# JialeTao/MRFA

Hardware: AMD Instinct MI355X
Metric: frames/sec (256x256 source+driving pair) fwd+bwd (higher is better)
Workload: dtype f32; 1 GPU; vox1.yaml MTIA (TokenPose_B) prior + DenseMotion + RaftFlow refinement, 256x256, bs=8/GPU, fwd+bwd+clip+Adam, train-mode BN, surrogate L1 loss; global_batch=8, parallelism=dp1, prior=mtia, background_predictor=False, sync_bn=False, launch=hipGraph, optimizer=FlatAdam (K20), mfma=bf16x6

## Files before the change

### mrfa_amd/build.py

```python
import glob
import os
import subprocess
import sys

HERE = os.path.dirname(os.path.abspath(__file__))
ROOT = os.path.dirname(HERE)
CSRC = os.path.join(HERE, "csrc")
LIBDIR = os.path.join(HERE, "_lib")
LIB = os.path.join(LIBDIR, "libmrfa_hip.so")
SOURCES = ["error.cpp", "conv_plan.hip", "conv_mfma.hip", "conv_split.hip", "conv_halo.hip", "conv_small.hip", "conv_lean.hip", "wgrad_mfma.hip", "wgrad_split.hip", "wgrad_halo.hip", "wgrad_small.hip", "wgrad_lean.hip", "conv_fewout.hip", "conv_fewout3.hip", "layout.hip", "pack_multi.hip", "norm.hip", "sample.hip", "elementwise.hip", "optim.hip", "tokenpose.hip", "attention_mfma.hip", "losses.hip", "prior.hip", "pose.hip"]
FLAGS = ["--offload-arch=gfx950", "-O3", "-std=c++17", "-fPIC", "-I" + os.path.join(ROOT, "include"), "-I" + CSRC,
         "-Wno-unused-result"]


def _stale(out, deps):
    if not os.path.exists(out):
        return True
    t = os.path.getmtime(out)
    return any(os.path.getmtime(d) > t for d in deps)


def build(force: bool = False, verbose: bool = True) -> str:
    os.makedirs(LIBDIR, exist_ok=True)
    hipcc = os.environ.get("HIPCC", "/opt/rocm/bin/hipcc")
    headers = [os.path.join(ROOT, "include", h) for h in ("mrfa_hip.h", "mrfa_hip_ext.h")] + sorted(glob.glob(os.path.join(CSRC, "*.h")))
    objs = []
    procs = []
    for src in SOURCES:
        sp = os.path.join(CSRC, src)
        if not os.path.exists(sp):
            raise FileNotFoundError(sp)
        obj = os.path.join(LIBDIR, os.path.splitext(src)[0] + ".o")
        objs.append(obj)
        if force or _stale(obj, [sp] + headers):
            cmd = [hipcc] + FLAGS + (["-x", "hip"] if src.endswith(".cpp") else []) + ["-c", sp, "-o", obj]
            if verbose:
                print("[mrfa_amd.build]", " ".join(cmd), flush=True)
            procs.append((src, subprocess.Popen(cmd)))
    for src, pr in procs:
        if pr.wait() != 0:
            raise RuntimeError(f"hipcc failed on {src}")
    if force or _stale(LIB, objs):
        cmd = [hipcc, "--offload-arch=gfx950", "-shared", "-fPIC", "-o", LIB] + objs
        if verbose:
            print("[mrfa_amd.build]", " ".join(cmd), flush=True)
        subprocess.check_call(cmd)
    return LIB


if __name__ == "__main__":
    build(force="--force" in sys.argv)
    print(LIB)
```

### mrfa_amd/csrc/common.h

```cpp
#pragma once
#include <hip/hip_runtime.h>
#include <stdio.h>
#include <string.h>
#include "mrfa_hip.h"

typedef float f32x16 __attribute__((ext_vector_type(16)));
typedef float f32x4 __attribute__((ext_vector_type(4)));

void mrfa_set_error(const char* fmt, ...);

struct MrfaTuning {
    int conv_small_env;
    int conv_small;
    int conv_halo, conv_halo_min_tiles, conv_halo_pr, conv_halo_phase, conv_halo_bn256, conv_halo_bn192, conv_halo_bn64_fill;
    int conv_lean, conv_lean_min_wgs, conv_lean_geo, gemm_lean;
    int wgrad_halo, wgrad_halo_min_wgs, wgrad_halo_target_wgs, wgrad_halo_phase, wgrad_lean;
    int conv_fewout3, attention_mfma, split_target_256;
};
extern MrfaTuning g_tune;

struct HaloGeo { int PR, BN; bool phase; };

enum class ConvFamily { lean, gemm_lean, small, halo, halo_dgrad, rows_split, rows_f32, refused };
struct ConvPlan {
    ConvFamily family;
    char error[256];
    long long M;
    int KT;
    int lean_geo, gemm_cfg, small_tm, small_tn;
    HaloGeo halo;
    int BM, BN, splitk;
    bool w8;
    bool fused;
    bool fin_in_launch;
    bool reads_w;
    int last_config;
    bool groups_ok, bst_ok, stride2_ok, mask_ok, phase_dgrad_ok;
};
ConvPlan plan_conv(const mrfa_conv_params& p);

enum class WgradFamily { lean, small, halo, tiled, refused };
struct WgradPlan {
    WgradFamily family;
    char error[192];
    long long M;
    bool lean, small;
    bool groups_ok, stride2_ok;
};
WgradPlan plan_wgrad(const mrfa_wgrad_params& p);

int mrfa_conv_split_launch(hipStream_t st, const mrfa_conv_params& p, int KT, long long M, int splitk, int BN);
bool mrfa_conv_halo_eligible(const mrfa_conv_params& p, HaloGeo* geo);
int mrfa_conv_halo_launch(hipStream_t st, const mrfa_conv_params& p, const HaloGeo& geo);
int mrfa_wgrad_split_launch(hipStream_t st, const mrfa_wgrad_params& p, dim3 grid, long long M, long long kps, int tiles_n, int nsplit, int inner,
                            int total_splits, int taps, long long partial_stride, int BM, int BN);

bool mrfa_wgrad_halo_eligible(const mrfa_wgrad_params& p);
int mrfa_wgrad_halo_launch(hipStream_t st, const mrfa_wgrad_params& p);

bool mrfa_fewout3_wgrad(hipStream_t st, const float* x, int ldx, int N, int H, int W, int Cin, const float* dy, int lddy, int Cout, int R, int pad,
                        float* dw, float* dbias, int* rc);

int mrfa_conv_lean_pick(const mrfa_conv_params& p);
int mrfa_conv_lean_launch(hipStream_t st, const mrfa_conv_params& p, int geo);
int mrfa_gemm_lean_pick(const mrfa_conv_params& p, long long M);
int mrfa_gemm_lean_launch(hipStream_t st, const mrfa_conv_params& p, long long M, int cfg);

bool mrfa_conv_small_eligible(const mrfa_conv_params& p, long long M);
int mrfa_conv_small_launch(hipStream_t st, const mrfa_conv_params& p, long long M, int tm, int tn);

bool mrfa_attention_mfma_ok(int d, int n, const void* qkv, int ld, const void* out, int ldo, const void* dout, int lddo, const void* dqkv, int lddq);
int mrfa_attention_fwd_mfma(hipStream_t st, const float* qkv, int ld, int B, int n, int heads, int d, float scale, float* out, int ldo, float* lse);
int mrfa_attention_bwd_mfma(hipStream_t st, const float* qkv, int ld, const float* out, int ldo, const float* dout, int lddo, const float* lse,
                            float* delta, int B, int n, int heads, int d, float scale, float* dqkv, int lddq);

bool mrfa_wgrad_lean_eligible(const mrfa_wgrad_params& p);
int mrfa_wgrad_lean_multi(hipStream_t st, const mrfa_wgrad_params* ps, int n, unsigned char* taken);

bool mrfa_wgrad_small_eligible(const mrfa_wgrad_params& p, long long M);
int mrfa_wgrad_small_launch(hipStream_t st, const mrfa_wgrad_params& p, long long M);

#define MRFA_CHECK_ARG(cond, ...)                      \
    do {                                               \
        if (!(cond)) {                                 \
            mrfa_set_error(__VA_ARGS__);               \
            return 1;                                  \
        }                                              \
    } while (0)

#define MRFA_CHECK_LAUNCH(name)                                                   \
    do {                                                                          \
        hipError_t e_ = hipGetLastError();                                        \
        if (e_ != hipSuccess) {                                                   \
            mrfa_set_error("%s: launch failed: %s", name, hipGetErrorString(e_)); \
            return 2;                                                             \
        }                                                                         \
    } while (0)

static inline bool aligned16(const void* p) { return (reinterpret_cast<uintptr_t>(p) & 15u) == 0; }
static inline int cdiv(long long a, long long b) { return (int)((a + b - 1) / b); }

static inline int stream_grid(long long work_items, int block) {
    long long g = (work_items + block - 1) / block;
    if (g < 1) g = 1;
    if (g > 256 * 16) g = 256 * 16;
    return (int)g;
}

__device__ __forceinline__ int xcd_tile_index() {
    const int per_xcd = (int)gridDim.x >> 3;
    return (int)(blockIdx.x & 7) * per_xcd + (int)(blockIdx.x >> 3);
}

__device__ __forceinline__ void chain_prio() {
    __builtin_amdgcn_s_setprio(3);
}

__device__ __forceinline__ int stat_group(const mrfa_conv_params& p, long long row, long long M) {
    return p.groups > 1 ? (int)(row / (M / p.groups)) : 0;
}
__device__ __forceinline__ double* stat_slot(const mrfa_conv_params& p, int group, unsigned slot) {
    return p.stats + ((size_t)group * MRFA_STATS_SLOTS + slot % MRFA_STATS_SLOTS) * 2 * p.Cout;
}
static inline long long group_rows(const mrfa_conv_params& p, long long M) {
    if (p.groups <= 1) return M;
    return (p.N % p.groups) == 0 ? M / p.groups : 0;
}

__device__ __forceinline__ bool splitk_last_arriver(unsigned* ticket, unsigned nsplit) {
    __shared__ unsigned s_sk_ticket;
    asm volatile("s_waitcnt vmcnt(0)" ::: "memory");
    __syncthreads();
    if (threadIdx.x == 0) s_sk_ticket = __hip_atomic_fetch_add(ticket, 1u, __ATOMIC_RELAXED, __HIP_MEMORY_SCOPE_AGENT);
    __syncthreads();
    return s_sk_ticket == nsplit - 1;
}

__device__ __forceinline__ bool fin_last_arriver(unsigned* counter, unsigned participants, int idx) {
    __shared__ unsigned s_fin_ticket;
    asm volatile("s_waitcnt vmcnt(0)" ::: "memory");
    __syncthreads();
    if (threadIdx.x == 0) {
        if (idx < 0) {
            s_fin_ticket = __hip_atomic_fetch_add(counter, 1u, __ATOMIC_RELAXED, __HIP_MEMORY_SCOPE_AGENT) == participants - 1;
        } else {
            const unsigned nsh = participants < 8u ? participants : 8u, sh = (unsigned)idx % nsh;
            const unsigned mine = participants / nsh + (sh < participants % nsh ? 1u : 0u);
            unsigned last = 0;
            if (__hip_atomic_fetch_add(counter + 1 + sh, 1u, __ATOMIC_RELAXED, __HIP_MEMORY_SCOPE_AGENT) == mine - 1)
                last = __hip_atomic_fetch_add(counter, 1u, __ATOMIC_RELAXED, __HIP_MEMORY_SCOPE_AGENT) == nsh - 1;
            s_fin_ticket = last;
        }
    }
    __syncthreads();
    return s_fin_ticket != 0;
}

__device__ __forceinline__ double fin_slot_sum(const double* first, size_t stride) {
    double v[MRFA_STATS_SLOTS];
#pragma unroll
    for (int s = 0; s < MRFA_STATS_SLOTS; ++s) v[s] = __hip_atomic_load(first + (size_t)s * stride, __ATOMIC_RELAXED, __HIP_MEMORY_SCOPE_AGENT);
    double t = 0.0;
#pragma unroll
    for (int s = 0; s < MRFA_STATS_SLOTS; ++s) t += v[s];
    return t;
}

__device__ __forceinline__ void fused_bn_finalize(const mrfa_conv_params& p, unsigned participants, int idx = -1, double* scratch = nullptr, int scratch_n = 0) {
    if (!fin_last_arriver(p.fin_counter, participants, idx)) return;
    const double cnt = (double)p.fin_count;
    const int G = p.groups > 1 ? p.groups : 1;
    const int C2 = 2 * p.Cout;
    const bool par = scratch != nullptr && scratch_n >= G * C2;
    if (par) {
        for (int o = threadIdx.x; o < G * C2; o += blockDim.x) scratch[o] = fin_slot_sum(p.stats + (size_t)(o / C2) * MRFA_STATS_SLOTS * C2 + o % C2, (size_t)C2);
        __syncthreads();
    }
    for (int c = threadIdx.x; c < p.Cout; c += blockDim.x) {
        float rm = p.fin_rmean ? p.fin_rmean[c] : 0.f, rv = p.fin_rmean ? p.fin_rvar[c] : 0.f;
        for (int g = 0; g < G; ++g) {
            const double* sg = p.stats + (size_t)g * MRFA_STATS_SLOTS * C2;
            const double t1 = par ? scratch[g * C2 + c] : fin_slot_sum(sg + c, (size_t)C2);
            const double t2 = par ? scratch[g * C2 + p.Cout + c] : fin_slot_sum(sg + p.Cout + c, (size_t)C2);
            const double m = t1 / cnt;
            double var = t2 / cnt - m * m;
            if (var < 0.0) var = 0.0;
            const float mean = (float)m, invstd = (float)(1.0 / sqrt(var + (double)p.fin_eps));
            const double unb = p.fin_count > 1 ? var * cnt / (cnt - 1.0) : var;
            rm = (1.f - p.fin_momentum) * rm + p.fin_momentum * mean;
            rv = (1.f - p.fin_momentum) * rv + p.fin_momentum * (float)unb;
            const float sc = p.fin_gamma[c] * invstd;
            const int gc = g * p.Cout + c;
            p.fin_scale[gc] = sc;
            p.fin_shift[gc] = p.fin_beta[c] - mean * sc;
            if (p.fin_mean) p.fin_mean[gc] = mean;
            if (p.fin_invstd) p.fin_invstd[gc] = invstd;
        }
        if (p.fin_rmean) { p.fin_rmean[c] = rm; p.fin_rvar[c] = rv; }
    }
}

__device__ __forceinline__ float wave_sum(float v) {
#pragma unroll
    for (int o = 32; o > 0; o >>= 1) v += __shfl_xor(v, o, 64);
    return v;
}
```

### mrfa_amd/csrc/conv_plan.hip

```cpp
#include "common.h"
#include <stdarg.h>
#include <stdlib.h>

namespace {
int env_int(const char* name, int dflt) { const char* e = getenv(name); return e ? atoi(e) : dflt; }
int env_on(const char* name) { const char* e = getenv(name); return !(e && e[0] == '0'); }
}

MrfaTuning g_tune = {
     env_on("MRFA_CONV_SMALL"),  1,
     env_on("MRFA_CONV_HALO"),  128,  0,  1,  1,
     1,  1,
     env_on("MRFA_CONV_LEAN"),  128,  -1,
     env_int("MRFA_GEMM_LEAN", 1),
     env_on("MRFA_WGRAD_HALO"),  192,  256,  1,
     env_on("MRFA_WGRAD_LEAN"),
     1,  env_on("MRFA_ATTENTION_MFMA"),  env_int("MRFA_SPLIT_TARGET_256", 1),
};

enum TuneKind { T_ON, T_INT, T_NONNEG, T_NONNEG_ON, T_LEVEL, T_POS };
static const struct { const char* key; int* field; TuneKind kind; } TUNING_KEYS[] = {
    {"conv_small", &g_tune.conv_small, T_ON},
    {"conv_halo", &g_tune.conv_halo, T_ON},
    {"conv_halo_min_tiles", &g_tune.conv_halo_min_tiles, T_INT},
    {"conv_halo_pr", &g_tune.conv_halo_pr, T_INT},
    {"conv_halo_phase", &g_tune.conv_halo_phase, T_ON},
    {"conv_halo_bn256", &g_tune.conv_halo_bn256, T_ON},
    {"conv_halo_bn192", &g_tune.conv_halo_bn192, T_ON},
    {"conv_halo_bn64_fill", &g_tune.conv_halo_bn64_fill, T_ON},
    {"conv_lean", &g_tune.conv_lean, T_ON},
    {"conv_lean_min_wgs", &g_tune.conv_lean_min_wgs, T_NONNEG},
    {"conv_lean_geo", &g_tune.conv_lean_geo, T_INT},
    {"gemm_lean", &g_tune.gemm_lean, T_LEVEL},
    {"wgrad_halo", &g_tune.wgrad_halo, T_ON},
    {"wgrad_halo_min_wgs", &g_tune.wgrad_halo_min_wgs, T_NONNEG},
    {"wgrad_halo_target_wgs", &g_tune.wgrad_halo_target_wgs, T_POS},
    {"wgrad_halo_phase", &g_tune.wgrad_halo_phase, T_NONNEG_ON},
    {"wgrad_lean", &g_tune.wgrad_lean, T_ON},
    {"conv_fewout3", &g_tune.conv_fewout3, T_ON},
    {"attention_mfma", &g_tune.attention_mfma, T_ON},
};

extern "C" int mrfa_set_tuning(const char* key, int value) {
    if (!key) return -1;
    for (const auto& k : TUNING_KEYS) {
        if (strcmp(key, k.key)) continue;
        const int prev = *k.field;
        switch (k.kind) {
            case T_ON: *k.field = value != 0; break;
            case T_INT: *k.field = value; break;
            case T_NONNEG: if (value >= 0) *k.field = value; break;
            case T_NONNEG_ON: if (value >= 0) *k.field = value != 0; break;
            case T_LEVEL: if (value >= 0) *k.field = value > 2 ? 2 : value; break;
            case T_POS: if (value > 0) *k.field = value; break;
        }
        return prev;
    }
    return -1;
}

namespace {
constexpr int BK = 32;

template <typename Plan>
Plan& refuse(Plan& c, const char* fmt, ...) {
    va_list ap;
    va_start(ap, fmt);
    vsnprintf(c.error, sizeof(c.error), fmt, ap);
    va_end(ap);
    c.family = decltype(c.family)::refused;
    return c;
}

void plan_rows(ConvPlan& c, const mrfa_conv_params& p, int mode) {
    const bool flat = p.kflat > 0;
    const long long M = c.M;
    const int KT = c.KT;
    const int nb = p.nbatch > 1 ? p.nbatch : 1;
    int BN = 128;
    {
        const int cands[4] = {128, 96, 64, 32};
        const double pen[4] = {1.0, 1.08, 1.16, 1.3};
        double best = 1e18;
        for (int i = 0; i < 4; ++i) {
            if (cands[i] == 96 && flat) continue;
            const double cost = (double)cdiv(p.Cout, cands[i]) * cands[i] * pen[i];
            if (cost < best) { best = cost; BN = cands[i]; }
        }
    }
    if (mode >= 1 && !flat && p.Cout >= 32) BN = p.Cout <= 64 ? 64 : 128;
    auto ntiles = [&](int bm, int bn) { return ((M + bm - 1) / bm) * cdiv(p.Cout, bn) * nb; };
    int BM = 128;
    if (BN == 96 && ntiles(128, 96) < 384) BN = 128;
    if (BN == 128) { if (M <= 32) BM = 32; else if (M <= 64) BM = 64; }
    else if (BN == 64 && M <= 64) BM = 64;
    int splitk = 1;
    const bool auto_split = (p.splitk == 0);
    if (p.splitk > 1) splitk = p.splitk;
    {
        const bool short_k_big_m = KT < 32 && M > 4096;
        const bool grouped_stats = p.groups > 1 && p.stats && !(p.sk_ticket && !p.accumulate);
        const int max_split = (auto_split && !short_k_big_m && !grouped_stats) ? (KT / 2 > 0 ? KT / 2 : 1) : 1;
        long long t = ntiles(BM, BN);
        if (t < 384 && !(short_k_big_m && t >= 128)) {
            const bool half_target = g_tune.split_target_256 && auto_split && p.sk_ticket && !p.accumulate && KT >= 72 && KT <= 320 && BM == 128 && t >= 8 && t <= 16;
            int want = (int)(((half_target ? 256 : 512) + t - 1) / t);
            if (auto_split) splitk = want <= max_split ? want : max_split;
            const int min_bm = (BN == 128) ? 32 : (BN == 64 ? 64 : 128);
            while (!half_target && ntiles(BM, BN) * splitk < 384 && BM > min_bm) {
                BM >>= 1;
                if (auto_split) {
                    t = ntiles(BM, BN);
                    want = (int)((512 + t - 1) / t);
                    splitk = want <= max_split ? want : max_split;
                }
            }
            if (splitk < 1) splitk = 1;
        }
    }
    bool w8 = false;
    if (p.tile) {
        BM = p.tile >> 16; BN = p.tile & 0x7fff; w8 = (p.tile & 0x8000) != 0;
        if (p.splitk >= 1) splitk = p.splitk;
    } else if (BM == 128 && BN == 128 && !flat) {
        w8 = true;
    }
    const bool split_operand = mode >= 1 && BM == 128 && (BN == 128 || BN == 64) && !flat;
    c.family = split_operand ? ConvFamily::rows_split : ConvFamily::rows_f32;
    c.BM = BM;
    c.BN = BN;
    c.w8 = w8;
    c.splitk = splitk;
    c.fused = splitk > 1 && p.sk_ticket && !p.accumulate;
    c.fin_in_launch = p.fin_scale && nb == 1 && (splitk == 1 || c.fused);
    c.reads_w = !(split_operand && mode != 3 && p.w_split);
    c.last_config = (BM << 16) | (BN << 4) | ((flat ? 1 : 0) << 1) | (splitk > 1 ? 1 : 0) | (split_operand ? 4 : 0);
}
}

ConvPlan plan_conv(const mrfa_conv_params& p) {
    ConvPlan c = {};
    const int mode = mrfa_get_mfma_mode();
    const bool flat = p.kflat > 0;
    c.M = (long long)p.N * p.Hout * p.Wout;
    c.KT = ((flat ? p.kflat : p.R * p.S * p.Cin) + BK - 1) / BK;
    c.splitk = 1;
    c.reads_w = true;
    c.fin_in_launch = p.fin_scale != nullptr;

    c.lean_geo = flat ? -1 : mrfa_conv_lean_pick(p);
    c.gemm_cfg = (flat || c.lean_geo >= 0) ? -1 : mrfa_gemm_lean_pick(p, c.M);
    const bool lean = c.lean_geo >= 0, gemm = c.gemm_cfg >= 0;
    const bool small = !lean && !gemm && g_tune.conv_small_env && g_tune.conv_small && mrfa_conv_small_eligible(p, c.M);
    const bool halo = !flat && mrfa_conv_halo_eligible(p, &c.halo);

    const long long rows = group_rows(p, c.M);
    c.groups_ok = p.groups <= 1 || !(p.stats || p.fin_scale || p.bst_x || p.in_scale) ||
                  (p.nbatch <= 1 && p.splitk <= 1 && rows > 0 &&
                   (lean || gemm || (!p.in_scale && ((rows % 128) == 0 || small || (p.stride <= 1 && halo)))));
    c.bst_ok = p.stats && !p.fin_scale && p.stride >= 0 && !flat && (lean || gemm || small);
    c.stride2_ok = p.stride == 2 && p.Hout == (p.Hin + 2 * p.pad - p.R) / 2 + 1 && p.Wout == (p.Win + 2 * p.pad - p.S) / 2 + 1 &&
                   (flat ? (!p.ups && p.nbatch <= 1 && p.splitk <= 1 && p.ktab) : small);
    c.mask_ok = halo;
    c.phase_dgrad_ok = p.ups == 2 && halo;

    if (!(p.x && p.w)) return refuse(c, "conv2d: null pointer");
    if (!(p.N > 0 && p.Cin > 0 && p.Cout > 0 && p.Hout > 0 && p.Wout > 0)) return refuse(c, "conv2d: bad sizes");
    if (!(p.R >= 1 && p.S >= 1 && p.R <= 15 && p.S <= 15)) return refuse(c, "conv2d: kernel size %dx%d unsupported", p.R, p.S);
    if (!((p.w_ld % 4) == 0 && aligned16(p.w))) return refuse(c, "conv2d: packed weight must be 16-B aligned, w_ld %% 4 == 0");
    if (!flat && (p.Cin % 32) != 0) return refuse(c, "conv2d: chunked mode needs Cin %% 32 == 0 (got %d); use flat mode", p.Cin);
    if (!flat && !((p.ldx % 4) == 0 && aligned16(p.x))) return refuse(c, "conv2d: chunked mode needs 16-B aligned x and ldx %% 4 == 0");
    if (!flat && p.in_scale && !(aligned16(p.in_scale) && aligned16(p.in_shift))) return refuse(c, "conv2d: in_scale/in_shift alignment");
    if (flat && !(p.ktab != nullptr && aligned16(p.ktab))) return refuse(c, "conv2d: flat mode needs a 16-B aligned ktab");
    if (lean) {
        c.family = ConvFamily::lean;
        c.reads_w = false;
        c.last_config = (32 << 16) | (32 << 4) | 4 | (1 << 27);
        return c;
    }
    if (gemm) {
        c.family = ConvFamily::gemm_lean;
        c.reads_w = false;
        c.last_config = (64 << 16) | (64 << 4) | 4 | (1 << 26);
        return c;
    }
    if (small) {
        c.family = ConvFamily::small;
        const int ncols = (p.Cout + 15) / 16 * 16;
        auto waves = [&](int wm, int wn) { return ((c.M + wm - 1) / wm) * ((ncols + wn - 1) / wn); };
        int tm = 2, tn = 2;
        if (waves(32, 32) < 2048) { tm = 1; tn = 2; }
        if (tm == 1 && waves(16, 32) < 2048) { tn = 1; }
        if (ncols % 32 != 0 && tn == 2 && ncols < 32) tn = 1;
        if (p.groups > 1 && tm == 2 && (rows % 128) != 0) tm = 1;
        c.small_tm = tm;
        c.small_tn = tn;
        c.last_config = (16 << 16) | (16 << 4) | 8;
        return c;
    }
    if (p.stride < 0 || p.stride > 2 || (p.stride == 2 && !(flat && !p.ups && p.nbatch <= 1)))
        return refuse(c, "conv2d: stride = %d is only implemented by the one-wave-per-tile kernel and by flat-K launches: ask mrfa_conv2d_stride_supported() first", p.stride);
    if (p.mask && !halo) return refuse(c, "conv2d: `mask` is only honoured by the patch-tiled kernel: ask mrfa_conv2d_mask_supported() first");
    if (p.ups == 2 && !halo)
        return refuse(c, "conv2d: ups = 2 (phase data gradient of a fused-upsample layer) is only implemented for the shapes mrfa_conv2d_phase_dgrad_supported() reports");
    if (halo) {
        c.family = p.ups == 2 ? ConvFamily::halo_dgrad : ConvFamily::halo;
        c.reads_w = false;
        c.last_config = (128 << 16) | ((p.Cout <= 64 ? 64 : 128) << 4) | 4 | (1 << 28);
        return c;
    }
    plan_rows(c, p, mode);
    return c;
}

WgradPlan plan_wgrad(const mrfa_wgrad_params& p) {
    WgradPlan c = {};
    const bool flat = p.kflat > 0;
    c.M = (long long)p.N * p.Hout * p.Wout;
    c.lean = mrfa_wgrad_lean_eligible(p);
    c.small = g_tune.conv_small_env && g_tune.conv_small && mrfa_wgrad_small_eligible(p, c.M);
    c.groups_ok = p.groups <= 1 || !p.in_scale || c.lean;
    c.stride2_ok = p.stride == 2 && p.Hout == (p.Hin + 2 * p.pad - p.R) / 2 + 1 && p.Wout == (p.Win + 2 * p.pad - p.S) / 2 + 1 && c.small;
    if (!(p.x && p.dy && p.dw)) return refuse(c, "wgrad: null pointer");
    if (!flat && !((p.ldx % 4) == 0 && aligned16(p.x))) return refuse(c, "wgrad: x must be a 16-B aligned view with ld %% 4 == 0");
    if (flat && !p.ktab) return refuse(c, "wgrad: flat mode needs ktab");
    if (!(c.M < (1ll << 31) - 64)) return refuse(c, "wgrad: too many pixels");
    if (p.in_scale && c.lean) { c.family = WgradFamily::lean; return c; }
    if (!c.groups_ok) return refuse(c, "wgrad: groups = %d with a prologue is only implemented where mrfa_conv2d_wgrad_groups_supported() says so", p.groups);
    if (c.small) { c.family = WgradFamily::small; return c; }
    if (p.stride > 1) return refuse(c, "wgrad: stride = %d is only implemented by the small-problem kernel: ask mrfa_conv2d_wgrad_stride_supported() first", p.stride);
    c.family = !flat && mrfa_wgrad_halo_eligible(p) ? WgradFamily::halo : WgradFamily::tiled;
    return c;
}

extern "C" int mrfa_conv2d_split_k(const mrfa_conv_params* p) {
    if (!p) return 1;
    if (p->splitk > 1) return p->splitk;
    const ConvPlan c = plan_conv(*p);
    return c.family == ConvFamily::refused ? 1 : c.splitk;
}

extern "C" int mrfa_conv2d_reads_fp32_weights(const mrfa_conv_params* p) {
    if (!p) return 1;
    const ConvPlan c = plan_conv(*p);
    return c.family == ConvFamily::refused || c.reads_w ? 1 : 0;
}

extern "C" int mrfa_conv2d_groups_supported(const mrfa_conv_params* p) { return p && plan_conv(*p).groups_ok ? 1 : 0; }
extern "C" int mrfa_conv2d_bwdstats_supported(const mrfa_conv_params* p) { return p && plan_conv(*p).bst_ok ? 1 : 0; }
extern "C" int mrfa_conv2d_stride_supported(const mrfa_conv_params* p) { return p && plan_conv(*p).stride2_ok ? 1 : 0; }
extern "C" int mrfa_conv2d_mask_supported(const mrfa_conv_params* p) { return p && plan_conv(*p).mask_ok ? 1 : 0; }
extern "C" int mrfa_conv2d_phase_dgrad_supported(const mrfa_conv_params* p) { return p && plan_conv(*p).phase_dgrad_ok ? 1 : 0; }

extern "C" int mrfa_conv2d_wgrad_stride_supported(const mrfa_wgrad_params* p) { return p && plan_wgrad(*p).stride2_ok ? 1 : 0; }
extern "C" int mrfa_conv2d_wgrad_groups_supported(const mrfa_wgrad_params* p) { return p && plan_wgrad(*p).groups_ok ? 1 : 0; }
extern "C" int mrfa_conv2d_wgrad_lean_supported(const mrfa_wgrad_params* p) { return p && plan_wgrad(*p).lean ? 1 : 0; }
```

### mrfa_amd/csrc/wgrad_small.hip

```cpp
#include <vector>
#include "common.h"

namespace {

typedef float f32x4v __attribute__((ext_vector_type(4)));
typedef float f32x2v __attribute__((ext_vector_type(2)));

struct SmallProblem {
    const float* x; const float* dy; float* dw; float* dbias;
    int ldx, ldy, Hin, Win, Hout, Wout, Cin, Cout, R, S, pad, stride;
    float alpha;
    int M, chunks_per_wave, nblk_ci, nblk, pow2_w , pow2_hw, workgroups, groups8 ;
};

template <bool SPATIAL, bool POW2, bool ROWS, int NT>
__device__ __forceinline__ void wgrad_small_body(const SmallProblem& p, const int g, const int tap, const int blk, float (*sacc)[16 * NT][16 * NT + 1], float* sbias) {
    typedef float VT __attribute__((ext_vector_type(NT)));
    constexpr int B = 16 * NT;
    const long long M = p.M;
    const int chunks_per_wave = p.chunks_per_wave, nblk_ci = p.nblk_ci, nblk = p.nblk, pow2_w = p.pow2_w, pow2_hw = p.pow2_hw;
    const int lane = threadIdx.x & 63, wave = threadIdx.x >> 6;
    const int li = lane & 15, kq = lane >> 4;
    const int co0 = (blk / nblk_ci) * B, ci0 = (blk % nblk_ci) * B;
    const int dr = tap / p.S - p.pad, ds = tap % p.S - p.pad;
    const int Mi = (int)M;
    const int range = (4 * g + wave) * chunks_per_wave * 16;
    const int HWo = p.Hout * p.Wout;
    const int wstride = p.stride > 1 ? p.stride : 1;

    if (threadIdx.x < B) sbias[threadIdx.x] = 0.f;
    __syncthreads();

    f32x4v acc[NT][NT];
#pragma unroll
    for (int t = 0; t < NT; ++t)
#pragma unroll
        for (int u = 0; u < NT; ++u) acc[t][u] = f32x4v{0.f, 0.f, 0.f, 0.f};
    float bsum[NT];
#pragma unroll
    for (int t = 0; t < NT; ++t) bsum[t] = 0.f;
    const VT vzero = {};
    const float* dyp = p.dy + co0 + NT * li;
    const float* xp = p.x + ci0 + NT * li;

    int dy_lane[4], x_lane[4];
#pragma unroll
    for (int j = 0; j < 4; ++j) {
        dy_lane[j] = (4 * j + kq) * p.ldy + co0 + NT * li;
        x_lane[j] = (4 * j + kq) * p.ldx + ci0 + NT * li;
    }

    auto load = [&](int m0c, VT (&a)[4], VT (&b)[4]) {
        if constexpr (ROWS) {
            int mc = __builtin_amdgcn_readfirstlane(m0c);
            mc = mc < Mi ? mc : Mi - 16;
            const float* dyb = p.dy + (size_t)mc * p.ldy;
#pragma unroll
            for (int j = 0; j < 4; ++j) a[j] = *reinterpret_cast<const VT*>(dyb + dy_lane[j]);
            if constexpr (!SPATIAL) {
                const float* xb = p.x + (size_t)mc * p.ldx;
#pragma unroll
                for (int j = 0; j < 4; ++j) b[j] = *reinterpret_cast<const VT*>(xb + x_lane[j]);
            } else {
                const int img = mc >> pow2_hw, rem = mc & ((1 << pow2_hw) - 1);
                const int oy = rem >> pow2_w, ox0 = rem & ((1 << pow2_w) - 1);
                const int iy = oy * wstride + dr;
                const bool row_ok = (unsigned)iy < (unsigned)p.Hin;
                const float* xrow0 = p.x + (size_t)((img * p.Hin + (row_ok ? iy : 0)) * p.Win) * p.ldx + ci0 + NT * li;
                const int ix0 = ox0 * wstride + ds;
#pragma unroll
                for (int j = 0; j < 4; ++j) {
                    const int ix = ix0 + (4 * j + kq) * wstride;
                    const bool inb = row_ok && (unsigned)ix < (unsigned)p.Win;
                    const int ixc = ix < 0 ? 0 : (ix >= p.Win ? p.Win - 1 : ix);
                    const VT bv = *reinterpret_cast<const VT*>(xrow0 + (size_t)ixc * p.ldx);
                    b[j] = inb ? bv : vzero;
                }
            }
            return;
        }
#pragma unroll
        for (int j = 0; j < 4; ++j) {
            const int mraw = m0c + 4 * j + kq;
            const bool ok = mraw < Mi;
            const int m = ok ? mraw : Mi - 1;
            const VT av = *reinterpret_cast<const VT*>(dyp + (size_t)m * p.ldy);
            a[j] = ok ? av : vzero;
            bool xok = ok;
            int xrow = m;
            if (SPATIAL) {
                int img, oy, ox;
                if (POW2) {
                    img = m >> pow2_hw;
                    const int rem = m & ((1 << pow2_hw) - 1);
                    oy = rem >> pow2_w;
                    ox = rem & ((1 << pow2_w) - 1);
                } else {
                    img = m / HWo;
                    const int rem = m - img * HWo;
                    oy = rem / p.Wout;
                    ox = rem - oy * p.Wout;
                }
                const int iy = oy * wstride + dr, ix = ox * wstride + ds;
                const bool inb = (unsigned)iy < (unsigned)p.Hin && (unsigned)ix < (unsigned)p.Win;
                xok = ok && inb;
                xrow = inb ? (img * p.Hin + iy) * p.Win + ix : img * p.Hin * p.Win;
            }
            const VT bv = *reinterpret_cast<const VT*>(xp + (size_t)xrow * p.ldx);
            b[j] = xok ? bv : vzero;
        }
    };
    auto compute = [&](const VT (&a)[4], const VT (&b)[4]) {
#pragma unroll
        for (int j = 0; j < 4; ++j) {
#pragma unroll
            for (int t = 0; t < NT; ++t) {
#pragma unroll
                for (int u = 0; u < NT; ++u) acc[t][u] = __builtin_amdgcn_mfma_f32_16x16x4f32(a[j][t], b[j][u], acc[t][u], 0, 0, 0);
                bsum[t] += a[j][t];
            }
        }
    };

    VT ra[4][4], rb[4][4];
    int nc = 0;
    if (range < Mi) {
        const int left = (Mi - range + 15) / 16;
        nc = left < chunks_per_wave ? left : chunks_per_wave;
    }
#pragma unroll
    for (int s = 0; s < 3; ++s) load(range + s * 16, ra[s], rb[s]);
    for (int c0 = 0; c0 < nc; c0 += 4) {
#pragma unroll
        for (int s = 0; s < 4; ++s) {
            load(range + (c0 + s + 3) * 16, ra[(s + 3) & 3], rb[(s + 3) & 3]);
            if (c0 + s < nc) compute(ra[s], rb[s]);
        }
    }
#pragma unroll
    for (int t = 0; t < NT; ++t)
#pragma unroll
        for (int u = 0; u < NT; ++u)
#pragma unroll
            for (int r = 0; r < 4; ++r)
                if (wave < 2) sacc[wave][NT * (kq * 4 + r) + t][NT * li + u] = acc[t][u][r];
    __syncthreads();
    if (wave >= 2) {
#pragma unroll
        for (int t = 0; t < NT; ++t)
#pragma unroll
            for (int u = 0; u < NT; ++u)
#pragma unroll
                for (int r = 0; r < 4; ++r) sacc[wave - 2][NT * (kq * 4 + r) + t][NT * li + u] += acc[t][u][r];
    }
    if (p.dbias && tap == 0 && ci0 == 0) {
#pragma unroll
        for (int t = 0; t < NT; ++t) {
            float v = bsum[t];
            v += __shfl_xor(v, 16, 64);
            v += __shfl_xor(v, 32, 64);
            if (kq == 0) atomicAdd(&sbias[NT * li + t], v);
        }
    }
    __syncthreads();
    float* dw = p.dw + ((size_t)tap * p.Cout + co0) * p.Cin + ci0;
    for (int i = threadIdx.x; i < B * B; i += 256) {
        const int r = i / B, c = i % B;
        if (co0 + r < p.Cout && ci0 + c < p.Cin) atomicAdd(dw + (size_t)r * p.Cin + c, p.alpha * (sacc[0][r][c] + sacc[1][r][c]));
    }
    if (p.dbias && tap == 0 && ci0 == 0 && threadIdx.x < B && co0 + threadIdx.x < p.Cout) atomicAdd(p.dbias + co0 + threadIdx.x, sbias[threadIdx.x]);
}

template <bool SPATIAL, bool POW2, bool ROWS, int NT>
__global__ __launch_bounds__(256) void wgrad_small_kernel(const SmallProblem p) {
    chain_prio();
    __shared__ float sacc[2][16 * NT][16 * NT + 1];
    __shared__ float sbias[16 * NT];
    const int T = p.R * p.S, bid = blockIdx.x;
    wgrad_small_body<SPATIAL, POW2, ROWS, NT>(p, bid / (p.nblk * T), (bid / p.nblk) % T, bid % p.nblk, sacc, sbias);
}

constexpr int SMALL_MULTI = 28;
struct SmallMulti {
    int n;
    int prefix[SMALL_MULTI + 1];
    SmallProblem d[SMALL_MULTI];
};

template <bool SPATIAL, bool POW2, bool ROWS, int NT>
__global__ __launch_bounds__(256) void wgrad_small_multi_kernel(const SmallMulti a) {
    chain_prio();
    __shared__ float sacc[2][16 * NT][16 * NT + 1];
    __shared__ float sbias[16 * NT];
    int lo = 0, hi = a.n;
    while (hi - lo > 1) {
        const int mid = (lo + hi) >> 1;
        if ((int)blockIdx.x >= a.prefix[mid]) lo = mid; else hi = mid;
    }
    const SmallProblem& p = a.d[lo];
    const int local = (int)blockIdx.x - a.prefix[lo];
    const int T = p.R * p.S, j = local >> 3;
    const int g = (((local & 7) - lo) & 7) * p.groups8 + j / (p.nblk * T);
    if ((long long)(4 * g) * p.chunks_per_wave * 16 >= p.M) return;
    wgrad_small_body<SPATIAL, POW2, ROWS, NT>(p, g, (j / p.nblk) % T, j % p.nblk, sacc, sbias);
}

constexpr int SMALL_VARIANTS = 7;
int small_problem(const mrfa_wgrad_params& p, long long M, SmallProblem* o) {
    const int T = p.R * p.S;
    constexpr bool rows_on = true, b64_on = true;
    const bool spatial0 = T > 1 || p.Hin != p.Hout || p.Win != p.Wout;
    auto lg2_ = [](int v) { int l = 0; while ((1 << l) < v) ++l; return (1 << l) == v ? l : -1; };
    const bool rows0 = rows_on && (M % 16) == 0 && (!spatial0 || (lg2_(p.Wout) >= 0 && lg2_(p.Hout) >= 0 && (p.Wout % 16) == 0));
    const bool b64 = b64_on && rows0 && (p.Cin % 64) == 0 && (p.Cout % 64) == 0 && (p.ldx % 4) == 0 && (p.ldy % 4) == 0 &&
                     (reinterpret_cast<uintptr_t>(p.x) & 15) == 0 && (reinterpret_cast<uintptr_t>(p.dy) & 15) == 0;
    const int Bk = b64 ? 64 : 32;
    const int nblk_ci = p.Cin / Bk, nblk = (p.Cout / Bk) * nblk_ci;
    const long long chunks = (M + 15) / 16;
    long long groups = (2048 + (long long)nblk * T * 4 - 1) / ((long long)nblk * T * 4);
    const long long max_groups = (chunks + 15) / 16;
    if (groups > max_groups) groups = max_groups;
    if (groups < 1) groups = 1;
    const int chunks_per_wave = (int)((chunks + groups * 4 - 1) / (groups * 4));
    groups = (chunks + (long long)chunks_per_wave * 4 - 1) / ((long long)chunks_per_wave * 4);
    auto lg2 = [](int v) { int l = 0; while ((1 << l) < v) ++l; return (1 << l) == v ? l : -1; };
    int pw = lg2(p.Wout), ph = lg2(p.Hout);
    if (ph < 0) pw = -1;
    const bool spatial = T > 1 || p.Hin != p.Hout || p.Win != p.Wout;
    o->x = p.x; o->dy = p.dy; o->dw = p.dw; o->dbias = p.dbias;
    o->ldx = p.ldx; o->ldy = p.ldy; o->Hin = p.Hin; o->Win = p.Win; o->Hout = p.Hout; o->Wout = p.Wout; o->Cin = p.Cin; o->Cout = p.Cout;
    o->R = p.R; o->S = p.S; o->pad = p.pad; o->stride = p.stride; o->alpha = p.alpha;
    o->M = (int)M; o->chunks_per_wave = chunks_per_wave; o->nblk_ci = nblk_ci; o->nblk = nblk;
    o->pow2_w = (spatial && pw >= 0) ? pw : 0; o->pow2_hw = (spatial && pw >= 0) ? pw + ph : 0;
    o->workgroups = (int)(groups * T * nblk);
    o->groups8 = (int)((groups + 7) / 8);
    const bool rows = rows0;
    if (!spatial) return rows ? (b64 ? 6 : 4) : 2;
    return pw >= 0 ? (rows ? (b64 ? 5 : 3) : 0) : 1;
}

}

bool mrfa_wgrad_small_eligible(const mrfa_wgrad_params& p, long long M) {
    if (p.kflat > 0 || p.ups || p.in_scale || p.nbatch > 1 || p.ksplit > 0 || p.stride > 2) return false;
    if ((p.Cin & 31) || (p.Cout & 31) || (p.ldx & 1) || (p.ldy & 1)) return false;
    if ((reinterpret_cast<uintptr_t>(p.x) & 7) || (reinterpret_cast<uintptr_t>(p.dy) & 7)) return false;
    if (M > 65536 || p.Cout > 640 || p.Cin > 640) return false;
    if (p.stride == 2) return true;
    if (p.Cout >= 128 && p.Cin >= 128 && M > 6144) return false;
    if (2.0 * (double)M * p.Cout * (double)p.Cin * p.R * p.S > 1.3e9) return false;
    return true;
}

int mrfa_wgrad_small_launch(hipStream_t st, const mrfa_wgrad_params& p, long long M) {
    SmallProblem sp;
    const int variant = small_problem(p, M, &sp);
    dim3 grid((unsigned)sp.workgroups);
    switch (variant) {
        case 0: hipLaunchKernelGGL((wgrad_small_kernel<true, true, false, 2>), grid, dim3(256), 0, st, sp); break;
        case 1: hipLaunchKernelGGL((wgrad_small_kernel<true, false, false, 2>), grid, dim3(256), 0, st, sp); break;
        case 2: hipLaunchKernelGGL((wgrad_small_kernel<false, false, false, 2>), grid, dim3(256), 0, st, sp); break;
        case 3: hipLaunchKernelGGL((wgrad_small_kernel<true, true, true, 2>), grid, dim3(256), 0, st, sp); break;
        case 4: hipLaunchKernelGGL((wgrad_small_kernel<false, false, true, 2>), grid, dim3(256), 0, st, sp); break;
        case 5: hipLaunchKernelGGL((wgrad_small_kernel<true, true, true, 4>), grid, dim3(256), 0, st, sp); break;
        default: hipLaunchKernelGGL((wgrad_small_kernel<false, false, true, 4>), grid, dim3(256), 0, st, sp); break;
    }
    MRFA_CHECK_LAUNCH("mrfa_conv2d_wgrad_nhwc(small)");
    return 0;
}

extern "C" int mrfa_conv2d_wgrad_multi(void* stream, const mrfa_wgrad_params* ps, int n) {
    MRFA_CHECK_ARG(n >= 0 && (n == 0 || ps), "wgrad_multi: bad args");
    hipStream_t st = (hipStream_t)stream;
    SmallMulti batch[SMALL_VARIANTS];
    for (int v = 0; v < SMALL_VARIANTS; ++v) { batch[v].n = 0; batch[v].prefix[0] = 0; }
    auto flush = [&](int v) -> int {
        SmallMulti& b = batch[v];
        if (b.n == 0) return 0;
        dim3 grid((unsigned)b.prefix[b.n]);
        switch (v) {
            case 0: hipLaunchKernelGGL((wgrad_small_multi_kernel<true, true, false, 2>), grid, dim3(256), 0, st, b); break;
            case 1: hipLaunchKernelGGL((wgrad_small_multi_kernel<true, false, false, 2>), grid, dim3(256), 0, st, b); break;
            case 2: hipLaunchKernelGGL((wgrad_small_multi_kernel<false, false, false, 2>), grid, dim3(256), 0, st, b); break;
            case 3: hipLaunchKernelGGL((wgrad_small_multi_kernel<true, true, true, 2>), grid, dim3(256), 0, st, b); break;
            case 4: hipLaunchKernelGGL((wgrad_small_multi_kernel<false, false, true, 2>), grid, dim3(256), 0, st, b); break;
            case 5: hipLaunchKernelGGL((wgrad_small_multi_kernel<true, true, true, 4>), grid, dim3(256), 0, st, b); break;
            default: hipLaunchKernelGGL((wgrad_small_multi_kernel<false, false, true, 4>), grid, dim3(256), 0, st, b); break;
        }
        MRFA_CHECK_LAUNCH("mrfa_conv2d_wgrad_multi");
        b.n = 0;
        return 0;
    };
    std::vector<unsigned char> taken((size_t)n, 0);
    if (n > 0) { const int rc = mrfa_wgrad_lean_multi(st, ps, n, taken.data()); if (rc) return rc; }
    for (int i = 0; i < n; ++i) {
        if (taken[i]) continue;
        const mrfa_wgrad_params& p = ps[i];
        MRFA_CHECK_ARG(p.x && p.dy && p.dw && p.N > 0 && p.Hout > 0 && p.Wout > 0, "wgrad_multi: problem %d: null pointer / bad sizes", i);
        const long long M = (long long)p.N * p.Hout * p.Wout;
        if (!plan_wgrad(p).small) {
            const int rc = mrfa_conv2d_wgrad_nhwc(stream, &p);
            if (rc) return rc;
            continue;
        }
        SmallProblem sp;
        const int v = small_problem(p, M, &sp);
        SmallMulti& b = batch[v];
        b.d[b.n] = sp;
        b.prefix[b.n + 1] = b.prefix[b.n] + sp.groups8 * 8 * (p.R * p.S) * sp.nblk;
        if (++b.n == SMALL_MULTI) { const int rc = flush(v); if (rc) return rc; }
    }
    for (int v = 0; v < SMALL_VARIANTS; ++v) { const int rc = flush(v); if (rc) return rc; }
    return 0;
}
```

Measured before the change: 101.8 pairs/s.

## Add batched bf16-split MFMA GEMM path for 1x1 weight gradients

Adds a new wgrad kernel family that treats 1x1 stride-1 convolution weight gradients as a GEMM over pixels. It stages dy and x chunks into LDS as split-bf16 pieces and accumulates with 32x32x16 MFMA, with K-split across workgroups and atomic accumulation into dw and dbias. Eligible problems are grouped by channel-tile variant into multi-problem launches, and this path runs ahead of the small/tiled paths in the multi-wgrad dispatcher. The trade-off is atomics on dw and bias, plus extra LDS and register pressure.

```diff
diff --git a/mrfa_amd/build.py b/mrfa_amd/build.py
--- a/mrfa_amd/build.py
+++ b/mrfa_amd/build.py
@@ -8,7 +8,7 @@
 CSRC = os.path.join(HERE, "csrc")
 LIBDIR = os.path.join(HERE, "_lib")
 LIB = os.path.join(LIBDIR, "libmrfa_hip.so")
-SOURCES = ["error.cpp", "conv_plan.hip", "conv_mfma.hip", "conv_split.hip", "conv_halo.hip", "conv_small.hip", "conv_lean.hip", "wgrad_mfma.hip", "wgrad_split.hip", "wgrad_halo.hip", "wgrad_small.hip", "wgrad_lean.hip", "conv_fewout.hip", "conv_fewout3.hip", "layout.hip", "pack_multi.hip", "norm.hip", "sample.hip", "elementwise.hip", "optim.hip", "tokenpose.hip", "attention_mfma.hip", "losses.hip", "prior.hip", "pose.hip"]
+SOURCES = ["error.cpp", "conv_plan.hip", "conv_mfma.hip", "conv_split.hip", "conv_halo.hip", "conv_small.hip", "conv_lean.hip", "wgrad_mfma.hip", "wgrad_split.hip", "wgrad_halo.hip", "wgrad_small.hip", "wgrad_lean.hip", "wgrad_gemm.hip", "conv_fewout.hip", "conv_fewout3.hip", "layout.hip", "pack_multi.hip", "norm.hip", "sample.hip", "elementwise.hip", "optim.hip", "tokenpose.hip", "attention_mfma.hip", "losses.hip", "prior.hip", "pose.hip"]
 FLAGS = ["--offload-arch=gfx950", "-O3", "-std=c++17", "-fPIC", "-I" + os.path.join(ROOT, "include"), "-I" + CSRC,
          "-Wno-unused-result"]
 
diff --git a/mrfa_amd/csrc/common.h b/mrfa_amd/csrc/common.h
--- a/mrfa_amd/csrc/common.h
+++ b/mrfa_amd/csrc/common.h
@@ -14,7 +14,7 @@
     int conv_small;
     int conv_halo, conv_halo_min_tiles, conv_halo_pr, conv_halo_phase, conv_halo_bn256, conv_halo_bn192, conv_halo_bn64_fill;
     int conv_lean, conv_lean_min_wgs, conv_lean_geo, gemm_lean;
-    int wgrad_halo, wgrad_halo_min_wgs, wgrad_halo_target_wgs, wgrad_halo_phase, wgrad_lean;
+    int wgrad_halo, wgrad_halo_min_wgs, wgrad_halo_target_wgs, wgrad_halo_phase, wgrad_lean, wgrad_gemm;
     int conv_fewout3, attention_mfma, split_target_256;
 };
 extern MrfaTuning g_tune;
@@ -45,6 +45,7 @@
     char error[192];
     long long M;
     bool lean, small;
+    bool gemm;
     bool groups_ok, stride2_ok;
 };
 WgradPlan plan_wgrad(const mrfa_wgrad_params& p);
@@ -76,6 +77,9 @@
 
 bool mrfa_wgrad_lean_eligible(const mrfa_wgrad_params& p);
 int mrfa_wgrad_lean_multi(hipStream_t st, const mrfa_wgrad_params* ps, int n, unsigned char* taken);
+
+bool mrfa_wgrad_gemm_eligible(const mrfa_wgrad_params& p);
+int mrfa_wgrad_gemm_multi(hipStream_t st, const mrfa_wgrad_params* ps, int n, unsigned char* taken);
 
 bool mrfa_wgrad_small_eligible(const mrfa_wgrad_params& p, long long M);
 int mrfa_wgrad_small_launch(hipStream_t st, const mrfa_wgrad_params& p, long long M);
diff --git a/mrfa_amd/csrc/conv_plan.hip b/mrfa_amd/csrc/conv_plan.hip
--- a/mrfa_amd/csrc/conv_plan.hip
+++ b/mrfa_amd/csrc/conv_plan.hip
@@ -14,7 +14,7 @@
      env_on("MRFA_CONV_LEAN"),  128,  -1,
      env_int("MRFA_GEMM_LEAN", 1),
      env_on("MRFA_WGRAD_HALO"),  192,  256,  1,
-     env_on("MRFA_WGRAD_LEAN"),
+     env_on("MRFA_WGRAD_LEAN"),  1,
      1,  env_on("MRFA_ATTENTION_MFMA"),  env_int("MRFA_SPLIT_TARGET_256", 1),
 };
 
@@ -37,6 +37,7 @@
     {"wgrad_halo_target_wgs", &g_tune.wgrad_halo_target_wgs, T_POS},
     {"wgrad_halo_phase", &g_tune.wgrad_halo_phase, T_NONNEG_ON},
     {"wgrad_lean", &g_tune.wgrad_lean, T_ON},
+    {"wgrad_gemm", &g_tune.wgrad_gemm, T_ON},
     {"conv_fewout3", &g_tune.conv_fewout3, T_ON},
     {"attention_mfma", &g_tune.attention_mfma, T_ON},
 };
@@ -218,6 +219,7 @@
     const bool flat = p.kflat > 0;
     c.M = (long long)p.N * p.Hout * p.Wout;
     c.lean = mrfa_wgrad_lean_eligible(p);
+    c.gemm = !c.lean && mrfa_wgrad_gemm_eligible(p);
     c.small = g_tune.conv_small_env && g_tune.conv_small && mrfa_wgrad_small_eligible(p, c.M);
     c.groups_ok = p.groups <= 1 || !p.in_scale || c.lean;
     c.stride2_ok = p.stride == 2 && p.Hout == (p.Hin + 2 * p.pad - p.R) / 2 + 1 && p.Wout == (p.Win + 2 * p.pad - p.S) / 2 + 1 && c.small;
diff --git a/mrfa_amd/csrc/wgrad_gemm.hip b/mrfa_amd/csrc/wgrad_gemm.hip
--- /dev/null
+++ b/mrfa_amd/csrc/wgrad_gemm.hip
@@ -0,0 +1,273 @@
+#include <stdlib.h>
+#include "mfma_bf16.h"
+
+namespace {
+
+constexpr int WG_MAXP = 24;
+
+struct GemmW {
+    const float* x; const float* dy; float* dw; float* dbias;
+    int ldx, ldy, M, Cin, Cout;
+    float alpha;
+    int G;
+    int Q;
+};
+struct GemmWMulti {
+    int n;
+    int prefix[WG_MAXP + 1];
+    GemmW p[WG_MAXP];
+};
+
+template <int TCO, int TCI, bool KS, int NP>
+__global__ __launch_bounds__(256) void wgrad_gemm_kernel(const GemmWMulti a) {
+    constexpr int NBO = KS ? 1 : 2 * TCO, NBI = KS ? 1 : 2 * TCI;
+    constexpr int PC = KS ? 64 : 32;
+    constexpr int BLK = PC * 64;
+    constexpr int NPC = NP == 6 ? 3 : (NP == 3 ? 2 : 1);
+    constexpr int PLANE = (NBO + NBI) * BLK;
+    constexpr int UPB = PC * 8 / 256;
+    constexpr int ND = NBO * UPB, NX = NBI * UPB;
+    extern __shared__ __attribute__((aligned(16))) unsigned char smem[];
+
+    const int tid = threadIdx.x, lane = tid & 63, wave = __builtin_amdgcn_readfirstlane(tid >> 6);
+    int pi = 0;
+    while (pi + 1 < a.n && (int)blockIdx.x >= a.prefix[pi + 1]) ++pi;
+    const GemmW& p = a.p[pi];
+    const int local = (int)blockIdx.x - a.prefix[pi];
+    const int nci = (p.Cin + 32 * NBI - 1) / (32 * NBI);
+    const int bg = local / p.G, jr = local - bg * p.G;
+    const int co0 = (bg / nci) * (32 * NBO), ci0 = (bg % nci) * (32 * NBI);
+    const int q0 = (int)((long long)jr * p.Q / p.G), q1 = (int)((long long)(jr + 1) * p.Q / p.G);
+    const bool want_bias = p.dbias != nullptr && ci0 == 0;
+
+    const int quad = tid & 7, px0 = tid >> 3;
+    f32x4 rd[ND], rx[NX], bsum[NBO];
+    unsigned okmask = 0;
+#pragma unroll
+    for (int b = 0; b < NBO; ++b) bsum[b] = f32x4{0.f, 0.f, 0.f, 0.f};
+    auto load_chunk = [&](int q) {
+        okmask = 0;
+#pragma unroll
+        for (int s = 0; s < UPB; ++s) {
+            const int m = q * PC + px0 + 32 * s;
+            const bool ok = m < p.M;
+            okmask |= ok ? (1u << s) : 0u;
+            const size_t row = (size_t)(ok ? m : p.M - 1);
+#pragma unroll
+            for (int b = 0; b < NBO; ++b) {
+                const int c = co0 + 32 * b < p.Cout ? co0 + 32 * b : 0;
+                rd[b * UPB + s] = *reinterpret_cast<const f32x4*>(p.dy + row * p.ldy + c + quad * 4);
+            }
+#pragma unroll
+            for (int b = 0; b < NBI; ++b) {
+                const int c = ci0 + 32 * b < p.Cin ? ci0 + 32 * b : 0;
+                rx[b * UPB + s] = *reinterpret_cast<const f32x4*>(p.x + row * p.ldx + c + quad * 4);
+            }
+        }
+    };
+    auto store_chunk = [&]() {
+        const f32x4 z = {0.f, 0.f, 0.f, 0.f};
+        unsigned char* const smD = smem;
+        unsigned char* const smX = smD + NBO * BLK;
+#pragma unroll
+        for (int j = 0; j < ND + NX; ++j) {
+            const bool isd = j < ND;
+            const int jj = isd ? j : j - ND, b = jj / UPB, s = jj % UPB;
+            const bool ok = ((okmask >> s) & 1u) && (isd ? co0 + 32 * b < p.Cout : ci0 + 32 * b < p.Cin);
+            const f32x4 v = ok ? (isd ? rd[jj] : rx[jj]) : z;
+            if (isd) bsum[b] += v;
+            u32x2 p1, p2, p3;
+            bf16_pieces<NP>(v, p1, p2, p3);
+            unsigned char* dst = (isd ? smD : smX) + b * BLK + (px0 + 32 * s) * 64 + quad * 8;
+            *reinterpret_cast<u32x2*>(dst) = p1;
+            if constexpr (NPC >= 2) *reinterpret_cast<u32x2*>(dst + PLANE) = p2;
+            if constexpr (NPC == 3) *reinterpret_cast<u32x2*>(dst + 2 * PLANE) = p3;
+        }
+    };
+
+    constexpr int AT = KS ? 1 : TCO, BT = KS ? 1 : TCI;
+    f32x16 acc[AT][BT];
+#pragma unroll
+    for (int i = 0; i < AT; ++i)
+#pragma unroll
+        for (int j = 0; j < BT; ++j)
+#pragma unroll
+            for (int r = 0; r < 16; ++r) acc[i][j][r] = 0.f;
+
+    const int l16 = lane & 15, grp16 = lane >> 4;
+    const int frag_off = (8 * (grp16 >> 1) + (l16 >> 2)) * 64 + (grp16 & 1) * 32 + (l16 & 3) * 8;
+    const int wco = KS ? 0 : (wave >> 1), wci = KS ? 0 : (wave & 1);
+    const int a_off = wco * TCO * BLK + frag_off, b_off = wci * TCI * BLK + frag_off;
+    auto compute = [&]() {
+        const unsigned char* const smD = smem;
+        const unsigned char* const smX = smD + NBO * BLK;
+#pragma unroll
+        for (int k = 0; k < (KS ? 1 : PC / 16); ++k) {
+            const int kk = KS ? wave : k;
+            bf16x8 af[AT][NPC], bfr[BT][NPC];
+#pragma unroll
+            for (int i = 0; i < AT; ++i)
+#pragma unroll
+                for (int pc = 0; pc < NPC; ++pc) af[i][pc] = tr_frag(smD + pc * PLANE + a_off + i * BLK + kk * 16 * 64);
+#pragma unroll
+            for (int j = 0; j < BT; ++j)
+#pragma unroll
+                for (int pc = 0; pc < NPC; ++pc) bfr[j][pc] = tr_frag(smX + pc * PLANE + b_off + j * BLK + kk * 16 * 64);
+#pragma unroll
+            for (int t = 6 - NP; t < 6; ++t)
+#pragma unroll
+                for (int i = 0; i < AT; ++i)
+#pragma unroll
+                    for (int j = 0; j < BT; ++j)
+                        acc[i][j] = __builtin_amdgcn_mfma_f32_32x32x16_bf16(af[i][PA[t]], bfr[j][PB[t]], acc[i][j], 0, 0, 0);
+        }
+    };
+
+    if (q0 >= q1) return;
+    load_chunk(q0);
+    for (int q = q0; q < q1; ++q) {
+        store_chunk();
+        __syncthreads();
+        if (q + 1 < q1) load_chunk(q + 1);
+        compute();
+        __syncthreads();
+    }
+
+    float* const red = reinterpret_cast<float*>(smem);
+    if (want_bias) {
+        if (tid < 32 * NBO) red[tid] = 0.f;
+        __syncthreads();
+#pragma unroll
+        for (int b = 0; b < NBO; ++b)
+#pragma unroll
+            for (int e = 0; e < 4; ++e) atomicAdd(&red[32 * b + quad * 4 + e], bsum[b][e]);
+        __syncthreads();
+        if (tid < 32 * NBO && co0 + tid < p.Cout) atomicAdd(p.dbias + co0 + tid, red[tid]);
+        __syncthreads();
+    }
+    if constexpr (KS) {
+        if (wave != 0) {
+#pragma unroll
+            for (int r = 0; r < 16; ++r) red[((wave - 1) * 16 + r) * 64 + lane] = acc[0][0][r];
+        }
+        __syncthreads();
+        if (wave != 0) return;
+#pragma unroll
+        for (int w = 0; w < 3; ++w)
+#pragma unroll
+            for (int r = 0; r < 16; ++r) acc[0][0][r] += red[(w * 16 + r) * 64 + lane];
+    }
+    const int half = lane >> 5;
+#pragma unroll
+    for (int i = 0; i < AT; ++i)
+#pragma unroll
+        for (int j = 0; j < BT; ++j) {
+            const int cob = co0 + (wco * TCO + i) * 32, ci = ci0 + (wci * TCI + j) * 32 + (lane & 31);
+            if (cob >= p.Cout || ci >= p.Cin) continue;
+#pragma unroll
+            for (int g = 0; g < 4; ++g)
+#pragma unroll
+                for (int e = 0; e < 4; ++e) {
+                    const int co = cob + 8 * g + 4 * half + e;
+                    atomicAdd(p.dw + (size_t)co * p.Cin + ci, p.alpha * acc[i][j][4 * g + e]);
+                }
+        }
+}
+
+constexpr size_t wg_lds(int tco, int tci, bool ks, int npc) {
+    const int nb = ks ? 2 : 2 * tco + 2 * tci, pc = ks ? 64 : 32;
+    const size_t st = (size_t)npc * nb * pc * 64, red = ks ? (size_t)3 * 16 * 64 * 4 : 0;
+    return st > red ? st : red;
+}
+
+constexpr int WG_VARIANTS = 5;
+int wg_variant(const mrfa_wgrad_params& p) {
+    if ((p.Cin % 64) || (p.Cout % 64)) return 0;
+    auto wide = [](int c) { return c >= 128 && ((c % 128) == 0 || c >= 512); };
+    return 1 + (wide(p.Cout) ? 2 : 0) + (wide(p.Cin) ? 1 : 0);
+}
+
+template <int TCO, int TCI, bool KS>
+int wg_launch(hipStream_t st, const GemmWMulti& m, int mode) {
+    dim3 grid((unsigned)m.prefix[m.n]);
+#define WG(NP_)                                                                                                                                    \
+    do {                                                                                                                                          \
+        constexpr size_t lds = wg_lds(TCO, TCI, KS, NP_ == 6 ? 3 : (NP_ == 3 ? 2 : 1));                                                            \
+        if constexpr (lds > 65536) {                                        \
+            static const hipError_t attr = hipFuncSetAttribute(reinterpret_cast<const void*>(&wgrad_gemm_kernel<TCO, TCI, KS, NP_>),               \
+                                                               hipFuncAttributeMaxDynamicSharedMemorySize, (int)lds);                             \
+            if (attr != hipSuccess) { mrfa_set_error("wgrad(gemm): %zu bytes of LDS refused: %s", lds, hipGetErrorString(attr)); return 2; }      \
+        }                                                                                                                                         \
+        hipLaunchKernelGGL((wgrad_gemm_kernel<TCO, TCI, KS, NP_>), grid, dim3(256), lds, st, m);                                                  \
+    } while (0)
+    if (mode == 3) WG(1);
+    else if (mode == 2) WG(3);
+    else WG(6);
+#undef WG
+    return 0;
+}
+
+}
+
+bool mrfa_wgrad_gemm_eligible(const mrfa_wgrad_params& p) {
+    const int mode = mrfa_get_mfma_mode();
+    if (!g_tune.wgrad_gemm || (mode != 1 && mode != 2 && mode != 3)) return false;
+    if (!(p.x && p.dy && p.dw && p.N > 0 && p.Hout > 0 && p.Wout > 0 && p.Cin > 0 && p.Cout > 0)) return false;
+    if (p.kflat > 0 || p.ups || p.R != 1 || p.S != 1 || p.pad != 0 || p.nbatch > 1 || p.ksplit > 0 || p.stride > 1 || p.in_scale) return false;
+    if (p.Hout != p.Hin || p.Wout != p.Win || (p.Cin % 32) != 0 || (p.Cout % 32) != 0) return false;
+    if ((p.ldx % 4) != 0 || !aligned16(p.x) || (p.ldy % 4) != 0 || !aligned16(p.dy)) return false;
+    if (p.ldx < p.Cin || p.ldy < p.Cout) return false;
+    return (long long)p.N * p.Hout * p.Wout < (1ll << 31) - 64;
+}
+
+int mrfa_wgrad_gemm_multi(hipStream_t st, const mrfa_wgrad_params* ps, int n, unsigned char* taken) {
+    const int mode = mrfa_get_mfma_mode();
+    for (int v = 0; v < WG_VARIANTS; ++v) {
+        GemmWMulti m;
+        m.n = 0;
+        int idx[WG_MAXP];
+        auto flush = [&]() -> int {
+            if (m.n == 0) return 0;
+            long long work = 0;
+            for (int k = 0; k < m.n; ++k) work += (long long)m.p[k].G * m.p[k].Q;
+            long long cpw = (work + 767) / 768;
+            if (cpw < 8) cpw = 8;
+            m.prefix[0] = 0;
+            for (int k = 0; k < m.n; ++k) {
+                GemmW& w = m.p[k];
+                const int blocks = w.G;
+                w.G = (int)((w.Q + cpw - 1) / cpw);
+                m.prefix[k + 1] = m.prefix[k] + w.G * blocks;
+            }
+            int rc = 0;
+            switch (v) {
+                case 0: rc = wg_launch<1, 1, true>(st, m, mode); break;
+                case 1: rc = wg_launch<1, 1, false>(st, m, mode); break;
+                case 2: rc = wg_launch<1, 2, false>(st, m, mode); break;
+                case 3: rc = wg_launch<2, 1, false>(st, m, mode); break;
+                default: rc = wg_launch<2, 2, false>(st, m, mode); break;
+            }
+            if (rc) return rc;
+            MRFA_CHECK_LAUNCH("mrfa_conv2d_wgrad_multi(gemm)");
+            for (int k = 0; k < m.n; ++k) taken[idx[k]] = 1;
+            m.n = 0;
+            return 0;
+        };
+        const int bco = v == 0 ? 32 : (v >= 3 ? 128 : 64), bci = v == 0 ? 32 : ((v == 2 || v == 4) ? 128 : 64), pc = v == 0 ? 64 : 32;
+        for (int i = 0; i < n; ++i) {
+            if (taken[i] || !mrfa_wgrad_gemm_eligible(ps[i]) || wg_variant(ps[i]) != v) continue;
+            const mrfa_wgrad_params& q = ps[i];
+            GemmW& w = m.p[m.n];
+            w.x = q.x; w.dy = q.dy; w.dw = q.dw; w.dbias = q.dbias;
+            w.ldx = q.ldx; w.ldy = q.ldy; w.M = q.N * q.Hout * q.Wout; w.Cin = q.Cin; w.Cout = q.Cout;
+            w.alpha = q.alpha;
+            w.Q = cdiv(w.M, pc);
+            w.G = cdiv(q.Cout, bco) * cdiv(q.Cin, bci);
+            idx[m.n] = i;
+            if (++m.n == WG_MAXP) { const int rc = flush(); if (rc) return rc; }
+        }
+        const int rc = flush();
+        if (rc) return rc;
+    }
+    return 0;
+}
diff --git a/mrfa_amd/csrc/wgrad_small.hip b/mrfa_amd/csrc/wgrad_small.hip
--- a/mrfa_amd/csrc/wgrad_small.hip
+++ b/mrfa_amd/csrc/wgrad_small.hip
@@ -293,6 +293,7 @@
     };
     std::vector<unsigned char> taken((size_t)n, 0);
     if (n > 0) { const int rc = mrfa_wgrad_lean_multi(st, ps, n, taken.data()); if (rc) return rc; }
+    if (n > 0) { const int rc = mrfa_wgrad_gemm_multi(st, ps, n, taken.data()); if (rc) return rc; }
     for (int i = 0; i < n; ++i) {
         if (taken[i]) continue;
         const mrfa_wgrad_params& p = ps[i];
```

Result: no change. 101.7 pairs/s, median of 2 (-0.0%).
